# aloe101/GNOT-Replication

Hardware: AMD Instinct MI355X
Metric: mesh points/sec (GNOT fwd+bwd, whole node) (higher is better)
Workload: dtype fp32; 1 GPU; configs[2]: synthetic 3-D mesh of 262,144 points, d=256, 8 experts, 8 heads, 1 input function (805 points), fp32 fwd+bwd; samples_per_gpu=1, input_function_points=805, hidden=256, experts=8, heads=8, blocks=4, mlp_layers=4, input_functions=1, geometry=fixed, moe_recompute=False, parallelism=single, step=pack+fwd+RelL2+bwd+AdamW (native loss, native flat AdamW) (hipGraph replay)

## Files before the change

gnot-replication_amd/csrc/wgrad.hip:

```cpp
#include <cstdlib>
#include <type_traits>

#include "gnot_common.h"
#include "gnot_kernels.h"
#include "x6_core.h"

namespace gnot {

typedef float f32x16 __attribute__((ext_vector_type(16)));

constexpr int kTile = 128;

GNOT_DEV int find_job(const int* __restrict__ prefix, int njobs, int idx) {
  int lo = 0, hi = njobs - 1;
  while (lo < hi) {
    const int mid = (lo + hi + 1) >> 1;
    if (prefix[mid] <= idx) lo = mid; else hi = mid - 1;
  }
  return lo;
}

constexpr int kX6Stage = 32;
constexpr int kX6Row = 40;
constexpr int kX6Piece = kTile * kX6Row;

#if defined(__HIP_DEVICE_COMPILE__)
#define GNOT_GLOBAL __attribute__((address_space(1)))
#else
#define GNOT_GLOBAL
#endif
typedef const float GNOT_GLOBAL* gfloat_ptr;
typedef const float2 GNOT_GLOBAL* gfloat2_ptr;

GNOT_DEV void x6_load8x2(float (&v)[2][8], const float* base, long ld, long prow, long pe, int f0, int ncols,
                         bool full, bool vec) {
  gfloat_ptr g = (gfloat_ptr)base;
  if (full && vec) {
    gfloat_ptr r = g + prow * ld + f0;
#pragma unroll
    for (int k = 0; k < 8; ++k) {
      const float2 x = *(gfloat2_ptr)(r + k * ld);
      v[0][k] = x.x;
      v[1][k] = x.y;
    }
    return;
  }
  const int c0 = min(f0, ncols - 1), c1 = min(f0 + 1, ncols - 1);
  const bool ok0 = f0 < ncols, ok1 = f0 + 1 < ncols;
#pragma unroll
  for (int k = 0; k < 8; ++k) {
    const long p = min(prow + k, pe - 1);
    const bool pv = prow + k < pe;
    gfloat_ptr r = g + p * ld;
    const float x0 = r[c0], x1 = r[c1];
    v[0][k] = (pv && ok0) ? x0 : 0.f;
    v[1][k] = (pv && ok1) ? x1 : 0.f;
  }
}

GNOT_DEV void x6_mfma6(const u32x4 (&a)[3], const u32x4 (&b)[3], f32x16& c) {
#define GNOT_MFMA32(X, Y) \
  c = __builtin_amdgcn_mfma_f32_32x32x16_bf16(__builtin_bit_cast(bf16x8, X), __builtin_bit_cast(bf16x8, Y), c, 0, 0, 0)
  GNOT_MFMA32(a[2], b[0]);
  GNOT_MFMA32(a[1], b[1]);
  GNOT_MFMA32(a[0], b[2]);
  GNOT_MFMA32(a[1], b[0]);
  GNOT_MFMA32(a[0], b[1]);
  GNOT_MFMA32(a[0], b[0]);
#undef GNOT_MFMA32
}
template <int NP>
GNOT_DEV void mfma_np(const u32x4 (&a)[NP], const u32x4 (&b)[NP], f32x16& c) {
  if constexpr (NP == 3) x6_mfma6(a, b, c);
  else c = __builtin_amdgcn_mfma_f32_32x32x16_bf16(__builtin_bit_cast(bf16x8, a[0]), __builtin_bit_cast(bf16x8, b[0]), c, 0, 0, 0);
}

template <int NP>
__global__ void __launch_bounds__(256) pgemm_x6_kernel(const WgradJob* __restrict__ jobs,
                                                       const int* __restrict__ prefix, int njobs,
                                                       float* __restrict__ slab) {
  __shared__ __attribute__((aligned(16))) unsigned short lds[2 * NP * kX6Piece];
  const int tid = threadIdx.x;
  const int lane = tid & 63, wave = tid >> 6;
  const int j = find_job(prefix, njobs, blockIdx.x);
  const WgradJob J = jobs[j];
  int t = blockIdx.x - prefix[j];
  const int split = t % J.splits;
  t /= J.splits;
  const int ti = t % J.tiles_i, to = t / J.tiles_i;
  const int chunk = ((J.P + J.splits - 1) / J.splits + kX6Stage - 1) / kX6Stage * kX6Stage;
  const long pb = (long)split * chunk;
  const long pe = min((long)J.P, pb + chunk);
  const int wo = wave >> 1, wi = wave & 1;
  const int r32 = lane & 31, h = lane >> 5;
  const int fp = lane, o = wave;
  const int fo = to * kTile + 2 * fp, fi = ti * kTile + 2 * fp;
  const bool tile_a = to * kTile + kTile <= J.out && (J.lddz & 1) == 0 && (reinterpret_cast<size_t>(J.dz) & 7) == 0;
  const bool tile_b = ti * kTile + kTile <= J.in && (J.ldx & 1) == 0 && (reinterpret_cast<size_t>(J.x) & 7) == 0;
  const bool want_db = (J.db != nullptr) && ti == 0;
  const bool gel = J.x_gelu != 0;

  f32x16 acc[2][2];
#pragma unroll
  for (int a = 0; a < 2; ++a)
#pragma unroll
    for (int b = 0; b < 2; ++b) acc[a][b] = f32x16{};
  float dbacc[2] = {0.f, 0.f};

  float ra[2][8], rb[2][8];
  auto load_stage = [&](long pbase) {
    const long prow = pbase + 8 * o;
    const bool full = prow + 7 < pe;
    x6_load8x2(ra, J.dz, J.lddz, prow, pe, fo, J.out, full, tile_a);
    x6_load8x2(rb, J.x, J.ldx, prow, pe, fi, J.in, full, tile_b);
  };

  if (pb < pe) load_stage(pb);
  for (long p0 = pb; p0 < pe; p0 += kX6Stage) {
    __syncthreads();
#pragma unroll
    for (int jf = 0; jf < 2; ++jf) {
      float vb[8];
#pragma unroll
      for (int k = 0; k < 8; ++k) {
        vb[k] = gel ? gelu(rb[jf][k]) : rb[jf][k];
        dbacc[jf] += ra[jf][k];
      }
      u32x4 pa[NP], pbv[NP];
      split8_np<NP>(ra[jf], pa);
      split8_np<NP>(vb, pbv);
      const int f = 2 * fp + jf;
#pragma unroll
      for (int q = 0; q < NP; ++q) {
        *reinterpret_cast<u32x4*>(lds + q * kX6Piece + f * kX6Row + 8 * o) = pa[q];
        *reinterpret_cast<u32x4*>(lds + (NP + q) * kX6Piece + f * kX6Row + 8 * o) = pbv[q];
      }
      asm volatile("" ::: "memory");
    }
    __syncthreads();
    if (p0 + kX6Stage < pe) load_stage(p0 + kX6Stage);
#pragma unroll
    for (int ks = 0; ks < 2; ++ks) {
      const int koff = 16 * ks + 8 * h;
      u32x4 af[2][NP], bf[2][NP];
#pragma unroll
      for (int a = 0; a < 2; ++a)
#pragma unroll
        for (int q = 0; q < NP; ++q) {
          af[a][q] = *reinterpret_cast<const u32x4*>(lds + q * kX6Piece + (wo * 64 + a * 32 + r32) * kX6Row + koff);
          bf[a][q] = *reinterpret_cast<const u32x4*>(lds + (NP + q) * kX6Piece + (wi * 64 + a * 32 + r32) * kX6Row + koff);
        }
#pragma unroll
      for (int a = 0; a < 2; ++a)
#pragma unroll
        for (int b = 0; b < 2; ++b) mfma_np<NP>(af[a], bf[b], acc[a][b]);
      asm volatile("" ::: "memory");
    }
  }

  const int ntile = J.tiles_o * J.tiles_i;
  const int tile = to * J.tiles_i + ti;
  float* S = slab + J.slab_off + ((long)split * ntile + tile) * (kTile * (kTile + 1));
#pragma unroll
  for (int a = 0; a < 2; ++a)
#pragma unroll
    for (int b = 0; b < 2; ++b)
#pragma unroll
      for (int r = 0; r < 16; ++r) {
        const int row = wo * 64 + a * 32 + (r & 3) + 8 * (r >> 2) + 4 * h;
        const int col = wi * 64 + b * 32 + r32;
        S[row * (kTile + 1) + col] = acc[a][b][r];
      }
  if (want_db) {
    __syncthreads();
    float* red = reinterpret_cast<float*>(lds);
    red[o * kTile + 2 * fp] = dbacc[0];
    red[o * kTile + 2 * fp + 1] = dbacc[1];
    __syncthreads();
    if (tid < kTile) S[tid * (kTile + 1) + kTile] = (red[tid] + red[kTile + tid]) + (red[2 * kTile + tid] + red[3 * kTile + tid]);
  }
}

constexpr int kWStage = 16;
constexpr int kWThreads = 512;
constexpr int w_threads(int tw) { return tw * 2; }
constexpr int w_piece(int tw) { return tw / 32 * 64; }
constexpr int w_buf(int np, int tw = 256) { return 2 * np * w_piece(tw); }
constexpr int kWRawSlot = 2 * 2 * 64;
constexpr int kWRawSlots = 2;
constexpr size_t w_lds_bytes(int np, int tw = 256) {
  return (2 * (size_t)w_buf(np, tw) + (size_t)(tw / 32) * kWRawSlots * kWRawSlot) * 16;
}

template <int OFF>
GNOT_DEV float lds_read_b32_off(unsigned addr) {
  float v;
  asm volatile("ds_read_b32 %0, %1 offset:%2" : "=v"(v) : "v"(addr), "n"(OFF) : "memory");
  return v;
}

template <int NP = 3, int TW = 256, bool SCK = false>
__global__ void __launch_bounds__(w_threads(TW)) pgemm_x6w_kernel(const WgradJob* __restrict__ jobs,
                                                                 const int* __restrict__ prefix, int njobs,
                                                                 float* __restrict__ slab,
                                                                 const int4* __restrict__ segs,
                                                                 const int* __restrict__ seg_start) {
  constexpr int NW = TW / 32;
  constexpr int FG = TW / 64;
  constexpr int WC = NW / 2;
  constexpr int RB = TW / 64;
  constexpr int kWPiece = w_piece(TW);
  extern __shared__ __attribute__((aligned(16))) u32x4 wl[];
  const int tid = threadIdx.x;
  const int lane = tid & 63, wave = __builtin_amdgcn_readfirstlane(tid >> 6);
  int k0 = 0, k1 = 1;
  if (segs != nullptr) { k0 = seg_start[blockIdx.x]; k1 = seg_start[blockIdx.x + 1]; }
  for (int kseg = k0; kseg < k1; ++kseg) {
  int j, split;
  long pb, pe;
  if (segs != nullptr) {
    const int4 sg = segs[kseg];
    j = sg.x; split = sg.y; pb = sg.z; pe = sg.w;
    if (kseg > k0) __syncthreads();
  } else {
    j = find_job(prefix, njobs, blockIdx.x);
    split = blockIdx.x - prefix[j];
    const int chunk = ((jobs[j].P + jobs[j].splits - 1) / jobs[j].splits + kWStage - 1) / kWStage * kWStage;
    pb = (long)split * chunk;
    pe = min((long)jobs[j].P, pb + chunk);
  }
  const WgradJob J = jobs[j];
  const int nst = pe > pb ? (int)((pe - pb + kWStage - 1) / kWStage) : 0;
  const int f = tid & (TW - 1), hh = tid / TW;
  const bool fa = f < J.out, fb = f < J.in;
  const int sdst = (f >> 5) * 64 + (f & 31) + 32 * hh;
  const int wr = wave / WC, wc = wave % WC;
  const int nrb = max(0, min(RB, (J.out - 32 * RB * wr + 31) / 32));
  const int ncb = max(0, min(2, (J.in - 64 * wc + 31) / 32));
  const bool full = nrb == RB && ncb == 2;
  const bool gel = J.x_gelu != 0;
  const bool scaled = SCK && J.scale != nullptr;

  f32x16 acc[RB][2];
#pragma unroll
  for (int a = 0; a < RB; ++a)
#pragma unroll
    for (int b = 0; b < 2; ++b) acc[a][b] = f32x16{};
  float dbacc = 0.f;
  float ra_raw[8], rb_raw[8];
  const long nsp = pe > pb ? pe - pb : 0;
  const rsrc_t rA = make_rsrc(J.dz + pb * J.lddz, (unsigned)(nsp * J.lddz * 4));
  const rsrc_t rB = make_rsrc(J.x + pb * J.ldx, (unsigned)(nsp * J.ldx * 4));
  const rsrc_t rS = make_rsrc(scaled ? J.scale + pb * J.ldscale : nullptr,
                              scaled && nsp > 0 ? (unsigned)(((nsp - 1) * J.ldscale + 1) * 4) : 0u);
  auto scale_voff = [&](int st) __attribute__((always_inline)) {
    int l = lane & 7;
    asm volatile("" : "+v"(l));
    return (st * kWStage + 8 * (wave / FG) + l) * (int)J.ldscale * 4;
  };
  auto scale_load = [&](int st) __attribute__((always_inline)) { return buf_load_f32(rS, scale_voff(st), 0); };
  auto scale_issue = [&](int st) __attribute__((always_inline)) {
    float v;
    asm volatile("buffer_load_dword %0, %1, %2, 0 offen" : "=v"(v) : "v"(scale_voff(st)), "s"(rS) : "memory");
    return v;
  };
  auto scale_of = [](float v, int k) __attribute__((always_inline)) {
    return __builtin_bit_cast(float, __builtin_amdgcn_readlane(__builtin_bit_cast(int, v), k));
  };
  const int fcol = 64 * (wave % FG) + 4 * (lane & 15);
  const int dvA = ((lane >> 4) * (int)J.lddz + fcol) * 4, dvB = ((lane >> 4) * (int)J.ldx + fcol) * 4;
  u32x4* const raw = wl + 2 * w_buf(NP, TW) + wave * kWRawSlots * kWRawSlot;
  auto raw_dma = [&](int st) __attribute__((always_inline)) {
    u32x4* dst = raw + (st & 1) * kWRawSlot;
    const unsigned p0 = (unsigned)(st * kWStage + 8 * (wave / FG));
#pragma unroll
    for (int i = 0; i < 2; ++i) {
      dma16(rA, dst + i * 64, dvA, (int)((p0 + 4 * i) * (unsigned)J.lddz * 4u));
      dma16(rB, dst + 128 + i * 64, dvB, (int)((p0 + 4 * i) * (unsigned)J.ldx * 4u));
    }
  };
  const unsigned raw_addr = (unsigned)(uintptr_t)(const __attribute__((address_space(3))) u32x4*)raw + 4u * lane;
  auto raw_read = [&](int st) __attribute__((always_inline)) {
    const unsigned a = raw_addr + (unsigned)((st & 1) * kWRawSlot * 16);
    ra_raw[0] = lds_read_b32_off<0>(a);    rb_raw[0] = lds_read_b32_off<2048>(a);
    ra_raw[1] = lds_read_b32_off<256>(a);  rb_raw[1] = lds_read_b32_off<2304>(a);
    ra_raw[2] = lds_read_b32_off<512>(a);  rb_raw[2] = lds_read_b32_off<2560>(a);
    ra_raw[3] = lds_read_b32_off<768>(a);  rb_raw[3] = lds_read_b32_off<2816>(a);
    ra_raw[4] = lds_read_b32_off<1024>(a); rb_raw[4] = lds_read_b32_off<3072>(a);
    ra_raw[5] = lds_read_b32_off<1280>(a); rb_raw[5] = lds_read_b32_off<3328>(a);
    ra_raw[6] = lds_read_b32_off<1536>(a); rb_raw[6] = lds_read_b32_off<3584>(a);
    ra_raw[7] = lds_read_b32_off<1792>(a); rb_raw[7] = lds_read_b32_off<3840>(a);
    asm volatile("s_waitcnt lgkmcnt(0)"
                 : "+v"(ra_raw[0]), "+v"(ra_raw[1]), "+v"(ra_raw[2]), "+v"(ra_raw[3]), "+v"(ra_raw[4]),
                   "+v"(ra_raw[5]), "+v"(ra_raw[6]), "+v"(ra_raw[7]), "+v"(rb_raw[0]), "+v"(rb_raw[1]),
                   "+v"(rb_raw[2]), "+v"(rb_raw[3]), "+v"(rb_raw[4]), "+v"(rb_raw[5]), "+v"(rb_raw[6]),
                   "+v"(rb_raw[7])::"memory");
  };
  auto stage_v = [&](int buf, auto GEL, auto SC, float sc) {
    float ra[8], vb[8];
#pragma unroll
    for (int k = 0; k < 8; ++k) {
      const float av = decltype(SC)::value ? mul_rn(ra_raw[k], scale_of(sc, k)) : ra_raw[k];
      ra[k] = fa ? av : 0.f;
      const float b = fb ? rb_raw[k] : 0.f;
      dbacc += ra[k];
      vb[k] = decltype(GEL)::value ? gelu(b) : b;
    }
    u32x4 pa[NP], pq[NP];
    split8_np<NP>(ra, pa);
    split8_np<NP>(vb, pq);
    u32x4* base = wl + buf * w_buf(NP, TW);
#pragma unroll
    for (int q = 0; q < NP; ++q) {
      base[q * kWPiece + sdst] = pa[q];
      base[(NP + q) * kWPiece + sdst] = pq[q];
    }
  };
  auto stage = [&](int buf, int st) {
    float sc = 0.f;
    if (scaled) {
      sc = scale_load(st);
      if (gel) stage_v(buf, std::true_type{}, std::true_type{}, sc);
      else stage_v(buf, std::false_type{}, std::true_type{}, sc);
    } else {
      if (gel) stage_v(buf, std::true_type{}, std::false_type{}, sc);
      else stage_v(buf, std::false_type{}, std::false_type{}, sc);
    }
  };
  auto compute = [&](int buf) {
    const u32x4* A = wl + buf * w_buf(NP, TW);
    const u32x4* Bm = A + NP * kWPiece;
    u32x4 bf[2][NP];
#pragma unroll
    for (int jb = 0; jb < 2; ++jb)
#pragma unroll
      for (int q = 0; q < NP; ++q) bf[jb][q] = Bm[q * kWPiece + (wc * 2 + jb) * 64 + lane];
#pragma unroll
    for (int ib = 0; ib < RB; ++ib) {
      if (ib >= nrb) break;
      u32x4 af[NP];
#pragma unroll
      for (int q = 0; q < NP; ++q) af[q] = A[q * kWPiece + (wr * RB + ib) * 64 + lane];
      if (ncb > 0) mfma_np<NP>(af, bf[0], acc[ib][0]);
      if (ncb > 1) mfma_np<NP>(af, bf[1], acc[ib][1]);
    }
  };
  auto lds_barrier = []() __attribute__((always_inline)) { asm volatile("s_waitcnt lgkmcnt(0)\n\ts_barrier" ::: "memory"); };

  if (nst > 0) {
    raw_dma(0);
    raw_dma(1);
    c2_wait_vm<4>();
    raw_read(0);
    raw_dma(2);
    stage(0, 0);
    lds_barrier();
    int buf = 0;
    auto fused = [&](int b, auto GEL, auto MASK, auto SC, float sc) {
      const u32x4* A = wl + b * w_buf(NP, TW);
      const u32x4* Bm = A + NP * kWPiece;
      u32x4 bf[2][NP], af[2][NP], pa[NP], pq[NP];
#pragma unroll
      for (int jb = 0; jb < 2; ++jb)
#pragma unroll
        for (int q = 0; q < NP; ++q) bf[jb][q] = Bm[q * kWPiece + (wc * 2 + jb) * 64 + lane];
#pragma unroll
      for (int q = 0; q < NP; ++q) af[0][q] = A[q * kWPiece + (wr * RB) * 64 + lane];
      float ra[8], vb[8];
      auto chunk = [&](int k) {
        const float av = decltype(SC)::value ? mul_rn(ra_raw[k], scale_of(sc, k)) : ra_raw[k];
        ra[k] = (!decltype(MASK)::value || fa) ? av : 0.f;
        dbacc += ra[k];
        const float bv = (!decltype(MASK)::value || fb) ? rb_raw[k] : 0.f;
        vb[k] = decltype(GEL)::value ? gelu(bv) : bv;
        asm volatile("" : "+v"(ra[k]), "+v"(vb[k]), "+v"(dbacc));
        if (k & 1) {
          split2_np<NP>(ra[k - 1], ra[k], pa, k >> 1);
          split2_np<NP>(vb[k - 1], vb[k], pq, k >> 1);
#pragma unroll
          for (int q = 0; q < NP; ++q) asm volatile("" : "+v"(pa[q][k >> 1]), "+v"(pq[q][k >> 1]));
        }
      };
      constexpr int CPG = 8 / (2 * RB);
#pragma unroll
      for (int ib = 0; ib < RB; ++ib) {
        if (ib + 1 < RB) {
#pragma unroll
          for (int q = 0; q < NP; ++q) af[(ib + 1) & 1][q] = A[q * kWPiece + (wr * RB + ib + 1) * 64 + lane];
        }
        mfma_np<NP>(af[ib & 1], bf[0], acc[ib][0]);
        __builtin_amdgcn_sched_barrier(0);
#pragma unroll
        for (int k = 0; k < CPG; ++k) chunk(CPG * 2 * ib + k);
        __builtin_amdgcn_sched_barrier(0);
        mfma_np<NP>(af[ib & 1], bf[1], acc[ib][1]);
        __builtin_amdgcn_sched_barrier(0);
#pragma unroll
        for (int k = 0; k < CPG; ++k) chunk(CPG * (2 * ib + 1) + k);
        __builtin_amdgcn_sched_barrier(0);
      }
      u32x4* base = wl + (b ^ 1) * w_buf(NP, TW);
#pragma unroll
      for (int q = 0; q < NP; ++q) {
        base[q * kWPiece + sdst] = pa[q];
        base[(NP + q) * kWPiece + sdst] = pq[q];
      }
    };
    auto run = [&](auto GEL, auto MASK, auto SC) {
      float scn = 0.f;
      if (decltype(SC)::value) {
        scn = scale_load(1);
        c2_wait_vm<4>();
      }
      for (int s = 0; s + 1 < nst; ++s) {
        const float sc = scn;
        if (!decltype(SC)::value) c2_wait_vm<4>();
        raw_read(s + 1);
        if (decltype(SC)::value) scn = scale_issue(s + 2);
        raw_dma(s + 3);
        fused(buf, GEL, MASK, SC, sc);
        lds_barrier();
        buf ^= 1;
        if (decltype(SC)::value) asm volatile("s_waitcnt vmcnt(4)" : "+v"(scn) :: "memory");
      }
    };
    if (full && scaled && gel && J.out >= TW && J.in >= TW) {
      run(std::true_type{}, std::false_type{}, std::true_type{});
    } else if (full && !scaled) {
      if (J.out >= TW && J.in >= TW) {
        if (gel) run(std::true_type{}, std::false_type{}, std::false_type{});
        else run(std::false_type{}, std::false_type{}, std::false_type{});
      } else {
        if (gel) run(std::true_type{}, std::true_type{}, std::false_type{});
        else run(std::false_type{}, std::true_type{}, std::false_type{});
      }
    } else {
      for (int s = 0; s + 1 < nst; ++s) {
        c2_wait_vm<4>();
        raw_read(s + 1);
        raw_dma(s + 3);
        compute(buf);
        stage(buf ^ 1, s + 1);
        lds_barrier();
        buf ^= 1;
      }
    }
    compute(buf);
    asm volatile("s_waitcnt vmcnt(0)" ::: "memory");
  }

  const WgradJob* jp = &J;
  if constexpr (SCK) {
    jp = jobs + j;
    asm volatile("" : "+s"(jp));
  }
  const WgradJob& JE = *jp;
  const int ntile = JE.tiles_o * JE.tiles_i;
  float* S0 = slab + JE.slab_off + (long)split * ntile * (kTile * (kTile + 1));
#pragma unroll
  for (int ib = 0; ib < RB; ++ib)
#pragma unroll
    for (int jb = 0; jb < 2; ++jb)
#pragma unroll
      for (int r = 0; r < 16; ++r) {
        const int row = wr * 32 * RB + ib * 32 + (r & 3) + 8 * (r >> 2) + 4 * (lane >> 5);
        const int col = wc * 64 + jb * 32 + (lane & 31);
        if (row < JE.out && col < JE.in)
          S0[((row >> 7) * JE.tiles_i + (col >> 7)) * (kTile * (kTile + 1)) + (row & 127) * (kTile + 1) + (col & 127)] =
              acc[ib][jb][r];
      }
  if (JE.db != nullptr) {
    float* red = reinterpret_cast<float*>(wl);
    __syncthreads();
    red[hh * TW + f] = dbacc;
    __syncthreads();
    if (tid < TW && f < JE.out)
      S0[((f >> 7) * JE.tiles_i) * (kTile * (kTile + 1)) + (f & 127) * (kTile + 1) + kTile] = red[f] + red[TW + f];
  }
  }
}

constexpr int kBStage = 32;
constexpr int kBSlots = 4;
constexpr int kBOpnd = kBStage * kB16Row;
constexpr int kBSlotBytes = 2 * kBOpnd;
constexpr size_t kBLds = (size_t)kBSlots * kBSlotBytes;

GNOT_DEV u32x2 lds_tr_b64(unsigned addr) {
  u32x2 v;
  asm volatile("ds_read_b64_tr_b16 %0, %1" : "=v"(v) : "v"(addr) : "memory");
  return v;
}

__global__ void __launch_bounds__(kWThreads) pgemm_b16_kernel(const WgradJob* __restrict__ jobs,
                                                             const int* __restrict__ prefix, int njobs,
                                                             float* __restrict__ slab, const int4* __restrict__ segs,
                                                             const int* __restrict__ seg_start) {
  extern __shared__ __attribute__((aligned(16))) u32x4 bl[];
  const int tid = threadIdx.x, lane = tid & 63;
  const int wave = __builtin_amdgcn_readfirstlane(tid >> 6);
  int k0 = 0, k1 = 1;
  if (segs != nullptr) { k0 = seg_start[blockIdx.x]; k1 = seg_start[blockIdx.x + 1]; }
  for (int kseg = k0; kseg < k1; ++kseg) {
  int j, split;
  long pb, pe;
  if (segs != nullptr) {
    const int4 sg = segs[kseg];
    j = sg.x; split = sg.y; pb = sg.z; pe = sg.w;
    if (kseg > k0) __syncthreads();
  } else {
    j = find_job(prefix, njobs, blockIdx.x);
    split = blockIdx.x - prefix[j];
    const int chunk = ((jobs[j].P + jobs[j].splits - 1) / jobs[j].splits + kBStage - 1) / kBStage * kBStage;
    pb = (long)split * chunk;
    pe = min((long)jobs[j].P, pb + chunk);
  }
  const WgradJob J = jobs[j];
  const int nst = pe > pb ? (int)((pe - pb + kBStage - 1) / kBStage) : 0;
  const int wr = wave >> 2, wc = wave & 3;
  const unsigned bytes = (unsigned)((pe > pb ? pe - pb : 0) * kB16Row);
  const long rb = pb * (kB16Row / 4);
  const rsrc_t rA = make_rsrc(J.dz + rb, bytes), rB = make_rsrc(J.x + rb, bytes);
  const int hi = lane >> 5;
  const int dvoff = hi * kB16Row + (((lane & 31) ^ (((2 * wave + hi) & 3) << 2)) * 16);
  auto dma_stage = [&](int s) __attribute__((always_inline)) {
    const unsigned p0 = (unsigned)(s * kBStage);
    u32x4* slot = bl + (s % kBSlots) * (kBSlotBytes / 16);
#pragma unroll
    for (int i = 0; i < 2; ++i) {
      const int row = 2 * wave + 16 * i;
      const int soff = (int)((p0 + (unsigned)row) * (unsigned)kB16Row);
      dma16(rA, slot + row * (kB16Row / 16), dvoff, soff);
      dma16(rB, slot + (kBOpnd + row * kB16Row) / 16, dvoff, soff);
    }
  };
  const int G = lane >> 4, q = (lane >> 2) & 3, pq = lane & 3;
  const unsigned lds0 = (unsigned)(uintptr_t)(const __attribute__((address_space(3))) u32x4*)bl;
  auto frag = [&](unsigned base, int m, int ks) {
    const unsigned a = base + (unsigned)((16 * ks + 8 * (G >> 1) + q) * kB16Row + (((m ^ q) * 4 + pq) * 16) + (G & 1) * 8);
    const u32x2 x0 = lds_tr_b64(a), x1 = lds_tr_b64(a + 4 * kB16Row);
    return u32x4{x0[0], x0[1], x1[0], x1[1]};
  };

  f32x16 acc[4][2];
#pragma unroll
  for (int a = 0; a < 4; ++a)
#pragma unroll
    for (int b = 0; b < 2; ++b) acc[a][b] = f32x16{};
  float dbacc = 0.f;
  for (int s = 0; s < 3 && s < nst; ++s) dma_stage(s);
  for (int s = 0; s < nst; ++s) {
    c2_sync_n(4 * min(2, nst - 1 - s));
    if (s + 3 < nst) dma_stage(s + 3);
    const unsigned base = lds0 + (unsigned)((s % kBSlots) * kBSlotBytes);
    u32x4 af[2][4], bf[2][2];
#pragma unroll
    for (int ks = 0; ks < 2; ++ks) {
#pragma unroll
      for (int ib = 0; ib < 4; ++ib) af[ks][ib] = frag(base, 4 * wr + ib, ks);
#pragma unroll
      for (int jb = 0; jb < 2; ++jb) bf[ks][jb] = frag(base + kBOpnd, 2 * wc + jb, ks);
    }
#pragma unroll
    for (int ks = 0; ks < 2; ++ks) {
      __builtin_amdgcn_sched_barrier(0);
      if (ks == 0)
        asm volatile("s_waitcnt lgkmcnt(12)" : "+v"(af[0][0]), "+v"(af[0][1]), "+v"(af[0][2]), "+v"(af[0][3]),
                     "+v"(bf[0][0]), "+v"(bf[0][1])::"memory");
      else
        asm volatile("s_waitcnt lgkmcnt(0)" : "+v"(af[1][0]), "+v"(af[1][1]), "+v"(af[1][2]), "+v"(af[1][3]),
                     "+v"(bf[1][0]), "+v"(bf[1][1])::"memory");
#pragma unroll
      for (int ib = 0; ib < 4; ++ib)
        if (ib == wc) {
          const u32x4 w = af[ks][ib];
#pragma unroll
          for (int d = 0; d < 4; ++d) dbacc += bf16_lo(w[d]) + bf16_hi(w[d]);
        }
#pragma unroll
      for (int ib = 0; ib < 4; ++ib)
#pragma unroll
        for (int jb = 0; jb < 2; ++jb)
          acc[ib][jb] = __builtin_amdgcn_mfma_f32_32x32x16_bf16(__builtin_bit_cast(bf16x8, af[ks][ib]),
                                                                __builtin_bit_cast(bf16x8, bf[ks][jb]), acc[ib][jb], 0,
                                                                0, 0);
    }
  }

  const int ntile = J.tiles_o * J.tiles_i;
  float* S0 = slab + J.slab_off + (long)split * ntile * (kTile * (kTile + 1));
#pragma unroll
  for (int ib = 0; ib < 4; ++ib)
#pragma unroll
    for (int jb = 0; jb < 2; ++jb)
#pragma unroll
      for (int r = 0; r < 16; ++r) {
        const int row = wr * 128 + ib * 32 + (r & 3) + 8 * (r >> 2) + 4 * (lane >> 5);
        const int col = wc * 64 + jb * 32 + (lane & 31);
        S0[((row >> 7) * J.tiles_i + (col >> 7)) * (kTile * (kTile + 1)) + (row & 127) * (kTile + 1) + (col & 127)] =
            acc[ib][jb][r];
      }
  dbacc += shfl_xor(dbacc, 32);
  if (J.db != nullptr && lane < 32) {
    const int f = wr * 128 + wc * 32 + lane;
    S0[((f >> 7) * J.tiles_i) * (kTile * (kTile + 1)) + (f & 127) * (kTile + 1) + kTile] = dbacc;
  }
  }
}

__global__ void __launch_bounds__(256) pgemm_reduce_kernel(const WgradJob* __restrict__ jobs,
                                                           const int* __restrict__ prefix, int njobs, int total,
                                                           const float* __restrict__ slab, int accumulate) {
  const int idx = blockIdx.x * 256 + threadIdx.x;
  if (idx >= total) return;
  const int j = find_job(prefix, njobs, idx);
  const WgradJob& J = jobs[j];
  int e = idx - prefix[j];
  const int ntile = J.tiles_o * J.tiles_i;
  const int tile = e / (kTile * (kTile + 1));
  e -= tile * (kTile * (kTile + 1));
  const int rl = e / (kTile + 1), cl = e % (kTile + 1);
  const int to = tile / J.tiles_i, ti = tile % J.tiles_i;
  const int row = to * kTile + rl;
  const bool isdb = cl == kTile;
  const int col = ti * kTile + cl;
  if (row >= J.out) return;
  if (isdb) {
    if (J.db == nullptr || ti != 0) return;
  } else if (col >= J.in) {
    return;
  }
  const float* S = slab + J.slab_off + (long)tile * (kTile * (kTile + 1)) + rl * (kTile + 1) + cl;
  const long sstride = (long)ntile * (kTile * (kTile + 1));
  float part[8] = {0.f, 0.f, 0.f, 0.f, 0.f, 0.f, 0.f, 0.f};
  int k = 0;
  for (; k + 8 <= J.splits; k += 8) {
    gfloat_ptr Sk = (gfloat_ptr)S + (long)k * sstride;
    asm volatile("" : "+v"(Sk));
#pragma unroll
    for (int u = 0; u < 8; ++u) part[u] += Sk[(long)u * sstride];
  }
  for (; k < J.splits; ++k) part[0] += S[(long)k * sstride];
  const float s = ((part[0] + part[1]) + (part[2] + part[3])) + ((part[4] + part[5]) + (part[6] + part[7]));
  float* dst = isdb ? (J.db + row) : (J.dW + (long)row * J.in + col);
  *dst = accumulate ? (*dst + s) : s;
}

hipError_t launch_wgrad(WgradKernel kind, const WgradTables& t, float* slab, int np, bool scaled, bool accumulate,
                        hipStream_t s) {
  if (t.njobs <= 0) return hipSuccess;
  if (np != 1 && np != 3) return hipErrorInvalidValue;
  if (scaled && !(kind == WgradKernel::Wide256 && np == 3)) return hipErrorInvalidValue;
  const bool ranged = kind == WgradKernel::Wide256 || kind == WgradKernel::B16Rows;
  if (t.segs != nullptr && !ranged) return hipErrorInvalidValue;
  const dim3 grid(t.total_wgs);
#define GNOT_WIDE(KERNEL, THREADS, LDS, ...)                                                                       \
  do {                                                                                                             \
    static bool attr = false;                                                                                      \
    if (!attr) {                                                                                                   \
      (void)hipFuncSetAttribute(reinterpret_cast<const void*>(KERNEL), hipFuncAttributeMaxDynamicSharedMemorySize, \
                                (int)(LDS));                                                                       \
      attr = true;                                                                                                 \
    }                                                                                                              \
    hipLaunchKernelGGL(KERNEL, grid, dim3(THREADS), LDS, s, t.jobs, t.wg_prefix, t.njobs, slab, __VA_ARGS__);      \
  } while (0)
  switch (kind) {
    case WgradKernel::Tile128:
      if (np == 1) hipLaunchKernelGGL(pgemm_x6_kernel<1>, grid, dim3(256), 0, s, t.jobs, t.wg_prefix, t.njobs, slab);
      else hipLaunchKernelGGL(pgemm_x6_kernel<3>, grid, dim3(256), 0, s, t.jobs, t.wg_prefix, t.njobs, slab);
      break;
    case WgradKernel::Wide256:
      if (scaled) GNOT_WIDE((pgemm_x6w_kernel<3, 256, true>), w_threads(256), w_lds_bytes(3, 256), t.segs, t.seg_start);
      else if (np == 1) GNOT_WIDE((pgemm_x6w_kernel<1, 256, false>), w_threads(256), w_lds_bytes(1, 256), t.segs, t.seg_start);
      else GNOT_WIDE((pgemm_x6w_kernel<3, 256, false>), w_threads(256), w_lds_bytes(3, 256), t.segs, t.seg_start);
      break;
    case WgradKernel::Wide128:
      if (np == 1) GNOT_WIDE((pgemm_x6w_kernel<1, 128, false>), w_threads(128), w_lds_bytes(1, 128), t.segs, t.seg_start);
      else GNOT_WIDE((pgemm_x6w_kernel<3, 128, false>), w_threads(128), w_lds_bytes(3, 128), t.segs, t.seg_start);
      break;
    case WgradKernel::B16Rows:
      GNOT_WIDE(pgemm_b16_kernel, kWThreads, kBLds, t.segs, t.seg_start);
      break;
  }
#undef GNOT_WIDE
  hipLaunchKernelGGL(pgemm_reduce_kernel, dim3((t.total_red + 255) / 256), dim3(256), 0, s, t.jobs, t.red_prefix,
                     t.njobs, t.total_red, (const float*)slab, accumulate ? 1 : 0);
  return hipGetLastError();
}

}
```

Before: 1.171 million points/s.

## Stagger global-load head in upper-half waves of weight-gradient GEMM

In the NP=3, TW=256 weight-gradient kernel, the upper half of the waves now issue their per-stage global wait, raw read and next DMA partway through the MFMA loop rather than before it. Those late waves compress their eight split/convert chunks into the MFMA groups that come after that point. The aim is to stop all waves stalling on vmcnt and issuing memory traffic at the same moment, so VMEM waits and DMA issue overlap with other waves' MFMA work. The cost is an uneven per-wave instruction schedule, extra template instantiations, and possible register pressure or LDS hazards if the timing assumptions are wrong.

```diff
diff --git a/gnot-replication_amd/csrc/wgrad.hip b/gnot-replication_amd/csrc/wgrad.hip
--- a/gnot-replication_amd/csrc/wgrad.hip
+++ b/gnot-replication_amd/csrc/wgrad.hip
@@ -190,6 +190,20 @@
 constexpr int kWRawSlots = 2;
 constexpr size_t w_lds_bytes(int np, int tw = 256) {
   return (2 * (size_t)w_buf(np, tw) + (size_t)(tw / 32) * kWRawSlots * kWRawSlot) * 16;
+}
+
+#ifndef GNOT_WSTAGGER
+#define GNOT_WSTAGGER 4
+#endif
+constexpr int kWStagger = GNOT_WSTAGGER;
+static_assert(kWStagger >= 1 && kWStagger <= 7, "the late waves stage all 8 points in the groups that are left");
+
+template <int I, int N, class F>
+GNOT_DEV void w_unroll(F&& f) {
+  if constexpr (I < N) {
+    f(std::integral_constant<int, I>{});
+    w_unroll<I + 1, N>(f);
+  }
 }
 
 template <int OFF>
@@ -356,7 +370,7 @@
     stage(0, 0);
     lds_barrier();
     int buf = 0;
-    auto fused = [&](int b, auto GEL, auto MASK, auto SC, float sc) {
+    auto fused = [&](int b, auto GEL, auto MASK, auto SC, auto LATE, float sc, auto&& head) {
       const u32x4* A = wl + b * w_buf(NP, TW);
       const u32x4* Bm = A + NP * kWPiece;
       u32x4 bf[2][NP], af[2][NP], pa[NP], pq[NP];
@@ -381,24 +395,33 @@
           for (int q = 0; q < NP; ++q) asm volatile("" : "+v"(pa[q][k >> 1]), "+v"(pq[q][k >> 1]));
         }
       };
-      constexpr int CPG = 8 / (2 * RB);
-#pragma unroll
-      for (int ib = 0; ib < RB; ++ib) {
+      constexpr int NG = 2 * RB;
+      constexpr int KS = decltype(LATE)::value ? kWStagger : 0;
+      auto chunks = [&](auto G) __attribute__((always_inline)) {
+        constexpr int g = decltype(G)::value;
+        if constexpr (g >= KS) {
+          constexpr int k0 = 8 * (g - KS) / (NG - KS), k1 = 8 * (g - KS + 1) / (NG - KS);
+#pragma unroll
+          for (int k = k0; k < k1; ++k) chunk(k);
+        }
+      };
+      w_unroll<0, RB>([&](auto IB) __attribute__((always_inline)) {
+        constexpr int ib = decltype(IB)::value;
+        if constexpr (decltype(LATE)::value && 2 * ib == KS) head();
         if (ib + 1 < RB) {
 #pragma unroll
           for (int q = 0; q < NP; ++q) af[(ib + 1) & 1][q] = A[q * kWPiece + (wr * RB + ib + 1) * 64 + lane];
         }
         mfma_np<NP>(af[ib & 1], bf[0], acc[ib][0]);
         __builtin_amdgcn_sched_barrier(0);
-#pragma unroll
-        for (int k = 0; k < CPG; ++k) chunk(CPG * 2 * ib + k);
+        chunks(std::integral_constant<int, 2 * ib>{});
         __builtin_amdgcn_sched_barrier(0);
+        if constexpr (decltype(LATE)::value && 2 * ib + 1 == KS) head();
         mfma_np<NP>(af[ib & 1], bf[1], acc[ib][1]);
         __builtin_amdgcn_sched_barrier(0);
-#pragma unroll
-        for (int k = 0; k < CPG; ++k) chunk(CPG * (2 * ib + 1) + k);
+        chunks(std::integral_constant<int, 2 * ib + 1>{});
         __builtin_amdgcn_sched_barrier(0);
-      }
+      });
       u32x4* base = wl + (b ^ 1) * w_buf(NP, TW);
 #pragma unroll
       for (int q = 0; q < NP; ++q) {
@@ -412,16 +435,27 @@
         scn = scale_load(1);
         c2_wait_vm<4>();
       }
-      for (int s = 0; s + 1 < nst; ++s) {
-        const float sc = scn;
-        if (!decltype(SC)::value) c2_wait_vm<4>();
-        raw_read(s + 1);
-        if (decltype(SC)::value) scn = scale_issue(s + 2);
-        raw_dma(s + 3);
-        fused(buf, GEL, MASK, SC, sc);
-        lds_barrier();
-        buf ^= 1;
-        if (decltype(SC)::value) asm volatile("s_waitcnt vmcnt(4)" : "+v"(scn) :: "memory");
+      auto loop = [&](auto LATE) __attribute__((always_inline)) {
+        for (int s = 0; s + 1 < nst; ++s) {
+          const float sc = scn;
+          auto head = [&]() __attribute__((always_inline)) {
+            if (!decltype(SC)::value) c2_wait_vm<4>();
+            raw_read(s + 1);
+            if (decltype(SC)::value) scn = scale_issue(s + 2);
+            raw_dma(s + 3);
+          };
+          if (!decltype(LATE)::value) head();
+          fused(buf, GEL, MASK, SC, LATE, sc, head);
+          lds_barrier();
+          buf ^= 1;
+          if (decltype(SC)::value) asm volatile("s_waitcnt vmcnt(4)" : "+v"(scn) :: "memory");
+        }
+      };
+      if constexpr (TW == 256 && NP == 3) {
+        if (wave >= NW / 2) loop(std::true_type{});
+        else loop(std::false_type{});
+      } else {
+        loop(std::false_type{});
       }
     };
     if (full && scaled && gel && J.out >= TW && J.in >= TW) {
```

Result: faster. 1.186 million points/s (median of 6 runs) (+1.3%).
